# Sunsett5/Noise-space-HMC

Measured on AMD Instinct MI355X. Metric: HMC leapfrog chain-steps/sec (256x256x3 FFHQ inpaint_random, U-Net score in the loop), higher is better.
Workload: dtype f32; 1 GPU; BASELINE configs[1]: FFHQ 256x256 inpaint_random sigma_0=0.05 tau=1.0 eps=0.05 timesteps=3, 64 chains per GPU, FFHQ U-Net architecture random-init fp32; chains_per_gpu=64, global_chains=64, score_chunk=64, parallelism=chains sharded over 1 rank(s), no data-path collective

## Files before the change

### noise-space-hmc_amd/csrc/wino_conv.hip

```cpp
#include "nhmc_common.h"

namespace {

typedef float f32x16 __attribute__((ext_vector_type(16)));
typedef float wc_v2f __attribute__((ext_vector_type(2)));

constexpr int WC_KBLK = 64;
constexpr int WC_ROWS = 4, WC_COLS = 64;
constexpr int WC_CHUNK = 8;
constexpr int WC_OPER = 16 * WC_CHUNK * 64;
constexpr int WC_LDS_BYTES = 4 * WC_OPER * 4;

#ifdef NHMC_WINO_STAMPS
__device__ unsigned long long* nhmc_wino_stamps;
__device__ int nhmc_wino_stamp_chunk;
#define WC_FENCE() __builtin_amdgcn_sched_barrier(0)
#define WC_T64(i) do { WC_FENCE(); t64[i] = __builtin_amdgcn_s_memtime(); WC_FENCE(); } while (0)
#define WC_R64(i) do { WC_FENCE(); t64[i] = __builtin_amdgcn_s_memrealtime(); WC_FENCE(); } while (0)
#define WC_T32(i) do { WC_FENCE(); const unsigned now_ = (unsigned)__builtin_amdgcn_s_memtime(); \
                       t32[i] = ch == stamp_ch ? now_ : t32[i]; WC_FENCE(); } while (0)
#else
#define WC_T64(i)
#define WC_R64(i)
#define WC_T32(i)
#endif

struct WinoArgs {
  const float* x; const float* U; const float* bias; const float* add; float* y;
  int C, K, H, W, row_blocks, col_blocks;
};

template <int TC, bool TAIL>
__global__ __launch_bounds__(256, 1) void k_conv3x3_wino(const WinoArgs a) {
  static_assert(TC == 32 || TC == 16 || TC == 8, "64 tiles as 32 / TC row pairs x TC columns");
  constexpr int BLK_ROWS = 128 / TC, BLK_COLS = 2 * TC;
  extern __shared__ __attribute__((aligned(16))) float lds[];
  const int tid = threadIdx.x, lane = tid & 63, wave = tid >> 6, lr = lane & 31, lh = lane >> 5;
  const int kh = wave & 1, th = wave >> 1;
  const int C = a.C, K = a.K, H = a.H, W = a.W, HW = H * W;
#ifdef NHMC_WINO_STAMPS
  unsigned long long t64[7] = {};
  unsigned t32[13] = {};
  const int stamp_ch = nhmc_wino_stamp_chunk < C / WC_CHUNK ? nhmc_wino_stamp_chunk : C / WC_CHUNK - 1;
#endif
  WC_T64(0);

  const int total = gridDim.x;
  int logical = blockIdx.x;
  if ((total & 7) == 0) logical = (logical & 7) * (total >> 3) + (logical >> 3);
  const int kblocks = TAIL ? (K + WC_KBLK - 1) / WC_KBLK : K / WC_KBLK;
  const int kb = logical % kblocks, sp = logical / kblocks;
  const bool tail_block = TAIL && kb == kblocks - 1;
  const bool idle = tail_block && __builtin_amdgcn_readfirstlane(kh) == 1;
  const bool u_row_ok = !(tail_block && tid >= 128);
  const int cb = sp % a.col_blocks, rb = (sp / a.col_blocks) % a.row_blocks, n = sp / (a.col_blocks * a.row_blocks);
  const int h0 = rb * BLK_ROWS, w0 = cb * BLK_COLS;

  const int lc = tid >> 5, ltx = tid & 31;
  unsigned voff[6][4];
  unsigned okmask = 0;
#pragma unroll
  for (int r = 0; r < 6; ++r) {
    const int row = h0 + 4 * (ltx / TC) - 1 + r;
    const bool rok = (unsigned)row < (unsigned)H;
#pragma unroll
    for (int s = 0; s < 4; ++s) {
      const int col = w0 + 2 * (ltx % TC) - 1 + s;
      const bool ok = rok && (unsigned)col < (unsigned)W;
      voff[r][s] = ok ? 4u * (unsigned)(lc * HW + row * W + col) : 0u;
      okmask |= ok ? 1u << (r * 4 + s) : 0u;
    }
  }
  const float* xn = a.x + (int64_t)n * C * HW;
  const char* un = reinterpret_cast<const char*>(a.U + (int64_t)kb * WC_KBLK * 16);
  const unsigned uoff = 16u * tid;
  const int uw = (tid & ~3) * 4 + (((tid & 3) ^ ((tid >> 4) & 3)) << 2);
  const int vw = (lc * 64 + ltx) * 16, vswz = (ltx >> 2) & 3;

  float xr[6][4];
  nhmc_v4f ur[8];
  auto load_one = [&](int ch, int i) {
    if (i < 24) {
      const char* xs = reinterpret_cast<const char*>(xn + (int64_t)ch * WC_CHUNK * HW);
      unsigned off = voff[i >> 2][i & 3];
      asm volatile("" : "+v"(off));
      xr[i >> 2][i & 3] = *reinterpret_cast<const float*>(xs + off);
    } else {
      const char* us = un + (int64_t)ch * WC_CHUNK * K * 64 + (int64_t)(i - 24) * K * 64;
      unsigned off = uoff;
      asm volatile("" : "+v"(off));
      if (!TAIL || u_row_ok) ur[i - 24] = *reinterpret_cast<const nhmc_v4f*>(us + off);
      else ur[i - 24] = nhmc_v4f{0.0f, 0.0f, 0.0f, 0.0f};
    }
  };
  auto issue_loads = [&](int ch, int first, int last) {
#pragma unroll
    for (int i = first; i < last; ++i) load_one(ch, i);
  };
  auto pin_patch = [&]() {
#pragma unroll
    for (int r = 0; r < 6; ++r)
#pragma unroll
      for (int s = 0; s < 4; ++s) asm volatile("" : "+v"(xr[r][s]));
  };
  auto d = [&](int r, int s) { return (okmask >> (r * 4 + s)) & 1u ? xr[r][s] : 0.0f; };
  auto stage_part = [&](int st, int b) {
    float* Us = lds + st * 2 * WC_OPER;
    float* Vs = Us + WC_OPER;
    float e[6];
#pragma unroll
    for (int r = 0; r < 6; ++r)
      e[r] = b == 0 ? d(r, 0) - d(r, 2) : b == 1 ? d(r, 1) + d(r, 2) : b == 2 ? d(r, 2) - d(r, 1) : d(r, 1) - d(r, 3);
#pragma unroll
    for (int ty = 0; ty < 2; ++ty) {
      const int r0 = 2 * ty;
      nhmc_v4f v;
      v.x = e[r0] - e[r0 + 2]; v.y = e[r0 + 1] + e[r0 + 2]; v.z = e[r0 + 2] - e[r0 + 1]; v.w = e[r0 + 1] - e[r0 + 3];
      *reinterpret_cast<nhmc_v4f*>(Vs + vw + ty * 32 * 16 + ((b ^ vswz) << 2)) = v;
    }
#pragma unroll
    for (int i = 2 * b; i < 2 * b + 2; ++i) *reinterpret_cast<nhmc_v4f*>(Us + uw + 1024 * i) = ur[i];
  };

  const int chunks = C / WC_CHUNK;
  f32x16 acc[16];
#pragma unroll
  for (int f = 0; f < 16; ++f)
#pragma unroll
    for (int r = 0; r < 16; ++r) acc[f][r] = 0.0f;

  const int swz = (lr >> 2) & 3;
  const int arow = (lh * 64 + kh * 32 + lr) * 16, brow = WC_OPER + (lh * 64 + th * 32 + lr) * 16;
  float av[2][8], bv[2][8];
  auto fetch = [&](int st, int u, float (&fa)[8], float (&fb)[8]) {
    const float* S = lds + st * 2 * WC_OPER + (u >> 1) * 2 * 64 * 16;
#pragma unroll
    for (int g = 0; g < 2; ++g) {
      const int go = ((2 * (u & 1) + g) ^ swz) << 2;
      const nhmc_v4f va = *reinterpret_cast<const nhmc_v4f*>(S + arow + go);
      const nhmc_v4f vb = *reinterpret_cast<const nhmc_v4f*>(S + brow + go);
      fa[4 * g + 0] = va.x; fa[4 * g + 1] = va.y; fa[4 * g + 2] = va.z; fa[4 * g + 3] = va.w;
      fb[4 * g + 0] = vb.x; fb[4 * g + 1] = vb.y; fb[4 * g + 2] = vb.z; fb[4 * g + 3] = vb.w;
    }
  };
  auto unit = [&](int u) {
#pragma unroll
    for (int j = 0; j < 8; ++j) {
      const int f = 8 * (u & 1) + j;
      if (!TAIL || !idle) acc[f] = __builtin_amdgcn_mfma_f32_32x32x2f32(av[u & 1][j], bv[u & 1][j], acc[f], 0, 0, 0);
    }
  };
  auto unit_loading = [&](int u, int cl) {
#pragma unroll
    for (int j = 0; j < 8; ++j) {
      const int f = 8 * (u & 1) + j;
      if (!TAIL || !idle) acc[f] = __builtin_amdgcn_mfma_f32_32x32x2f32(av[u & 1][j], bv[u & 1][j], acc[f], 0, 0, 0);
      if (u == 7) issue_loads(cl, (3 * j) / 2, (3 * j + 3) / 2);
      if (u == 0 && j < 6) issue_loads(cl, 12 + 2 * j, 14 + 2 * j);
      if (u == 0 && j >= 6) issue_loads(cl, 18 + j, 19 + j);
      if (u == 1 && (j & 1) == 0) issue_loads(cl, 26 + j / 2, 27 + j / 2);
      if (u == 2 && (j == 0 || j == 2)) issue_loads(cl, 30 + j / 2, 31 + j / 2);
      __builtin_amdgcn_sched_barrier(0);
    }
  };

  issue_loads(0, 0, 32);
#pragma unroll
  for (int b = 0; b < 4; ++b) stage_part(0, b);
  __syncthreads();
  WC_T64(1);
  int cl = 1 < chunks ? 1 : 0;
  issue_loads(cl, 0, 12);
  fetch(0, 0, av[0], bv[0]);
  int ch = 0, st = 0;
  WC_T64(2);
  WC_R64(5);
  do {
#pragma unroll
    for (int u = 0; u < 7; ++u) {
      WC_T32(u);
      fetch(st, u + 1, av[(u + 1) & 1], bv[(u + 1) & 1]);
      __builtin_amdgcn_sched_barrier(0);
      if (u < 3) unit_loading(u, cl);
      else unit(u);
      if (u == 3) {
        WC_T32(7);
        pin_patch();
        WC_T32(8);
      }
      if (u >= 3) stage_part(st ^ 1, u - 3);
    }
    WC_T32(9);
    __syncthreads();
    WC_T32(10);
    st ^= 1;
    cl = ch + 2 < chunks ? ch + 2 : chunks - 1;
    WC_T32(11);
    fetch(st, 0, av[0], bv[0]);
    __builtin_amdgcn_sched_barrier(0);
    unit_loading(7, cl);
    WC_T32(12);
  } while (++ch < chunks);
  WC_T64(3);
  WC_R64(6);

  if (TAIL && idle) return;
  const int oh = h0 + 4 * (lr / TC) + 2 * th, ow = w0 + 2 * (lr % TC);
  const bool has_bias = a.bias != nullptr, has_add = a.add != nullptr;
  const int k0 = kb * WC_KBLK + kh * 32 + 4 * lh;
  const bool odd = lr & 1;
  const int64_t at0 = (((int64_t)n * K + k0) * H + oh) * W + ow + (odd ? W - 2 : 0);
  float bc[16];
  nhmc_v4f ad[16];
#pragma unroll
  for (int r = 0; r < 16; ++r) {
    bc[r] = 0.0f;
    ad[r] = nhmc_v4f{0.0f, 0.0f, 0.0f, 0.0f};
  }
  if (has_bias) {
#pragma unroll
    for (int r = 0; r < 16; ++r) bc[r] = a.bias[k0 + (r & 3) + 8 * (r >> 2)];
  }
  if (has_add) {
#pragma unroll
    for (int r = 0; r < 16; ++r)
      ad[r] = *reinterpret_cast<const nhmc_v4f*>(a.add + at0 + (int64_t)((r & 3) + 8 * (r >> 2)) * HW);
  }
  auto neighbour = [](float v) {
    return __int_as_float(__builtin_amdgcn_update_dpp(0, __float_as_int(v), 0xB1, 0xF, 0xF, false));
  };
  __builtin_amdgcn_sched_barrier(0);
#pragma unroll
  for (int r = 0; r < 16; ++r) {
    float t[2][4];
#pragma unroll
    for (int b = 0; b < 4; ++b) {
      t[0][b] = (acc[4 * b + 0][r] + acc[4 * b + 1][r]) + acc[4 * b + 2][r];
      t[1][b] = (acc[4 * b + 1][r] - acc[4 * b + 2][r]) - acc[4 * b + 3][r];
    }
    wc_v2f o[2];
#pragma unroll
    for (int i = 0; i < 2; ++i) {
      o[i].x = (t[i][0] + t[i][1]) + t[i][2];
      o[i].y = (t[i][1] - t[i][2]) - t[i][3];
      o[i].x = has_bias ? o[i].x + bc[r] : o[i].x;
      o[i].y = has_bias ? o[i].y + bc[r] : o[i].y;
    }
    const wc_v2f keep = odd ? o[1] : o[0], send = odd ? o[0] : o[1];
    const wc_v2f got = {neighbour(send.x), neighbour(send.y)};
    nhmc_v4f v;
    v.x = odd ? got.x : keep.x; v.y = odd ? got.y : keep.y; v.z = odd ? keep.x : got.x; v.w = odd ? keep.y : got.y;
    if (has_add) v += ad[r];
    __builtin_nontemporal_store(v, reinterpret_cast<nhmc_v4f*>(a.y + at0 + (int64_t)((r & 3) + 8 * (r >> 2)) * HW));
  }
  WC_T64(4);
#ifdef NHMC_WINO_STAMPS
  if (nhmc_wino_stamps && lane == 0) {
    unsigned long long* out = nhmc_wino_stamps + ((size_t)blockIdx.x * 4 + wave) * 24;
#pragma unroll
    for (int i = 0; i < 7; ++i) out[i] = t64[i];
#pragma unroll
    for (int i = 0; i < 13; ++i) out[7 + i] = t32[i];
  }
#endif
}

__global__ __launch_bounds__(NHMC_BLOCK) void k_wino_weights(const float* __restrict__ w, float* __restrict__ U, int C, int K,
                                                             int backward) {
  const int CI = backward ? K : C, KO = backward ? C : K;
  const int idx = blockIdx.x * NHMC_BLOCK + threadIdx.x;
  if (idx >= CI * KO) return;
  const int ci = idx / KO, ko = idx % KO;
  const float* g = w + (int64_t)(backward ? ci * C + ko : ko * C + ci) * 9;
  float t[4][3];
#pragma unroll
  for (int s = 0; s < 3; ++s) {
    const float g0 = g[backward ? 8 - s : s], g1 = g[backward ? 5 - s : 3 + s], g2 = g[backward ? 2 - s : 6 + s];
    t[0][s] = g0; t[1][s] = 0.5f * ((g0 + g1) + g2); t[2][s] = 0.5f * ((g0 - g1) + g2); t[3][s] = g2;
  }
  nhmc_v4f u[4];
#pragma unroll
  for (int r = 0; r < 4; ++r) {
    u[0][r] = t[r][0];
    u[1][r] = 0.5f * ((t[r][0] + t[r][1]) + t[r][2]);
    u[2][r] = 0.5f * ((t[r][0] - t[r][1]) + t[r][2]);
    u[3][r] = t[r][2];
  }
#pragma unroll
  for (int b = 0; b < 4; ++b) reinterpret_cast<nhmc_v4f*>(U + (int64_t)idx * 16)[b] = u[b];
}

template <int TC, int KM = WC_KBLK>
int wc_covers_tc(int64_t n, int64_t c, int64_t k, int64_t h, int64_t w) {
  constexpr int ROWS = 128 / TC, COLS = 2 * TC;
  if (n <= 0 || c < WC_CHUNK || c % WC_CHUNK || k < KM || k % KM || h < ROWS || h % ROWS || w < COLS || w % COLS)
    return 0;
  if (TC != 32 && w != COLS) return 0;
  if (c > 65536 || k > 65536 || h * w > (1 << 24)) return 0;
  return n * (h / ROWS) * (w / COLS) * ((k + WC_KBLK - 1) / WC_KBLK) < (int64_t)1 << 31;
}

int wc_covers(int64_t n, int64_t c, int64_t k, int64_t h, int64_t w) { return wc_covers_tc<32>(n, c, k, h, w); }

int wc_narrow_covers(int64_t n, int64_t c, int64_t k, int64_t h, int64_t w) {
  return w == 32 ? wc_covers_tc<16>(n, c, k, h, w) : w == 16 ? wc_covers_tc<8>(n, c, k, h, w) : 0;
}

int wc_k32_covers(int64_t n, int64_t c, int64_t k, int64_t h, int64_t w) {
  return w == 32 ? wc_covers_tc<16, 32>(n, c, k, h, w) : w == 16 ? wc_covers_tc<8, 32>(n, c, k, h, w)
                                                                 : wc_covers_tc<32, 32>(n, c, k, h, w);
}

static_assert(WC_ROWS == 128 / 32 && WC_COLS == 2 * 32, "the wide geometry");

struct WcRow { int backward, c, k, res; };

template <int N>
int wc_listed(const WcRow (&table)[N], int backward, int c, int k, int h) {
  for (const WcRow& r : table)
    if (r.backward == (backward != 0) && r.c == c && r.k == k && r.res == h) return 1;
  return 0;
}

template <int TC, bool TAIL = false>
int wc_launch(const float* x, const float* u, const float* bias, const float* add, float* y, int n, int c, int k, int h, int w,
              nhmc_stream_t stream) {
  static bool attr_set[64] = {};
  int dev = 0;
  (void)hipGetDevice(&dev);
  if (dev < 0 || dev >= 64 || !attr_set[dev]) {
    if (hipFuncSetAttribute(reinterpret_cast<const void*>(&k_conv3x3_wino<TC, TAIL>), hipFuncAttributeMaxDynamicSharedMemorySize,
                            WC_LDS_BYTES) != hipSuccess)
      return NHMC_ERR_LAUNCH;
    if (dev >= 0 && dev < 64) attr_set[dev] = true;
  }
  const WinoArgs a{x, u, bias, add, y, c, k, h, w, h / (128 / TC), w / (2 * TC)};
  const int64_t blocks = (int64_t)n * a.row_blocks * a.col_blocks * ((k + WC_KBLK - 1) / WC_KBLK);
  NHMC_LAUNCH((k_conv3x3_wino<TC, TAIL>), dim3((unsigned)blocks), dim3(256), WC_LDS_BYTES, nhmc_s(stream), a);
  return nhmc_launch_status();
}

}

extern "C" int nhmc_conv3x3_wino_covers(int n, int c, int k, int h, int w) { return wc_covers(n, c, k, h, w); }
extern "C" int nhmc_conv3x3_wino_narrow_covers(int n, int c, int k, int h, int w) { return wc_narrow_covers(n, c, k, h, w); }

extern "C" int nhmc_conv3x3_wino_prefers(int backward, int n, int c, int k, int h, int w) {
  if (!wc_covers(n, c, k, h, w) || h != w) return 0;
  static const WcRow network[] = {
      {0, 128, 128, 256},
      {1, 128, 128, 256},
      {0, 256, 128, 256},
      {1, 128, 256, 256},
      {0, 128, 128, 128},
      {1, 128, 128, 128},
      {0, 256, 128, 128},
      {1, 128, 256, 128},
      {0, 256, 256, 128},
      {1, 256, 256, 128},
      {0, 384, 128, 128},
      {1, 128, 384, 128},
      {0, 128, 128, 64},
      {1, 128, 128, 64},
      {0, 128, 256, 64},
      {1, 256, 128, 64},
      {0, 256, 256, 64},
      {1, 256, 256, 64},
      {0, 384, 256, 64},
      {1, 256, 384, 64},
      {0, 512, 256, 64},
      {1, 256, 512, 64},
  };
  static const WcRow elsewhere[] = {
      {0, 384, 128, 256},
      {1, 128, 384, 256},
      {0, 128, 256, 128},
      {1, 256, 128, 128},
      {0, 384, 256, 128},
      {1, 256, 384, 128},
      {0, 512, 256, 128},
      {1, 256, 512, 128},
      {0, 256, 512, 64},
      {1, 512, 256, 64},
      {0, 512, 512, 64},
      {1, 512, 512, 64},
      {0, 768, 256, 64},
      {1, 256, 768, 64},
      {0, 1024, 512, 64},
      {1, 512, 1024, 64},
  };
  static const WcRow latent[] = {
      {0, 448, 448, 64},
      {0, 256, 256, 256},
      {1, 256, 256, 256},
      {0, 512, 512, 128},
      {1, 512, 512, 128},
  };
  return wc_listed(network, backward, c, k, h) || wc_listed(elsewhere, backward, c, k, h) || wc_listed(latent, backward, c, k, h);
}

extern "C" int nhmc_conv3x3_wino_narrow_prefers(int backward, int n, int c, int k, int h, int w) {
  if (!wc_narrow_covers(n, c, k, h, w) || h != w) return 0;
  static const WcRow network[] = {
      {0, 256, 256, 32},
      {1, 256, 256, 32},
      {0, 512, 256, 32},
      {1, 256, 512, 32},
      {0, 512, 512, 32},
      {1, 512, 512, 32},
      {0, 768, 256, 32},
      {1, 256, 768, 32},
      {0, 256, 256, 16},
      {1, 256, 256, 16},
      {0, 256, 512, 16},
      {1, 512, 256, 16},
      {0, 512, 512, 16},
      {1, 512, 512, 16},
      {0, 768, 512, 16},
      {1, 512, 768, 16},
      {0, 1024, 512, 16},
      {1, 512, 1024, 16},
  };
  static const WcRow latent[] = {
      {0, 224, 448, 32},
      {0, 448, 448, 32},
      {0, 672, 448, 32},
      {0, 896, 448, 32},
      {0, 1120, 448, 32},
      {0, 896, 896, 16},
  };
  return wc_listed(network, backward, c, k, h) || wc_listed(latent, backward, c, k, h);
}

extern "C" int nhmc_conv3x3_wino_k32_covers(int n, int c, int k, int h, int w) { return wc_k32_covers(n, c, k, h, w); }

extern "C" int nhmc_conv3x3_wino_k32_prefers(int backward, int n, int c, int k, int h, int w) {
  if (!wc_k32_covers(n, c, k, h, w) || h != w || k % WC_KBLK == 0) return 0;
  static const WcRow latent[] = {
      {0, 224, 224, 64},
      {0, 448, 224, 64},
      {0, 672, 224, 64},
      {0, 672, 672, 32},
      {0, 448, 672, 16},
      {0, 672, 672, 16},
      {0, 1120, 672, 16},
      {0, 1344, 672, 16},
      {0, 1568, 672, 16},
  };
  return wc_listed(latent, backward, c, k, h);
}

extern "C" int nhmc_wino_weights(const float* weight, float* u, int backward, int channels_in, int channels_out,
                                 nhmc_stream_t stream) {
  if (!weight || !u || (backward != 0 && backward != 1) || channels_in <= 0 || channels_out <= 0) return NHMC_ERR_ARG;
  if (channels_in > 65536 || channels_out > 65536) return NHMC_ERR_SHAPE;
  if (!nhmc_aligned16(u)) return NHMC_ERR_ALIGN;
  const int pairs = channels_in * channels_out;
  NHMC_LAUNCH(k_wino_weights, dim3((unsigned)((pairs + NHMC_BLOCK - 1) / NHMC_BLOCK)), dim3(NHMC_BLOCK), 0, nhmc_s(stream), weight,
              u, channels_in, channels_out, backward);
  return nhmc_launch_status();
}

extern "C" int nhmc_conv3x3_wino(const float* x, const float* u, const float* bias, const float* add, float* y, int n, int c,
                                 int k, int h, int w, int stride, int padding, nhmc_stream_t stream) {
  if (!x || !u || !y || y == x || (add && add == x)) return NHMC_ERR_ARG;
  if (stride != 1 || padding != 1 || !wc_covers(n, c, k, h, w)) return NHMC_ERR_SHAPE;
  if (!nhmc_aligned16(x) || !nhmc_aligned16(u) || !nhmc_aligned16(y) || !nhmc_aligned16(add)) return NHMC_ERR_ALIGN;
  return wc_launch<32>(x, u, bias, add, y, n, c, k, h, w, stream);
}

extern "C" int nhmc_conv3x3_wino_narrow(const float* x, const float* u, const float* bias, const float* add, float* y, int n,
                                        int c, int k, int h, int w, int stride, int padding, nhmc_stream_t stream) {
  if (!x || !u || !y || y == x || (add && add == x)) return NHMC_ERR_ARG;
  if (stride != 1 || padding != 1 || !wc_narrow_covers(n, c, k, h, w)) return NHMC_ERR_SHAPE;
  if (!nhmc_aligned16(x) || !nhmc_aligned16(u) || !nhmc_aligned16(y) || !nhmc_aligned16(add)) return NHMC_ERR_ALIGN;
  return w == 32 ? wc_launch<16>(x, u, bias, add, y, n, c, k, h, w, stream)
                 : wc_launch<8>(x, u, bias, add, y, n, c, k, h, w, stream);
}

extern "C" int nhmc_conv3x3_wino_k32(const float* x, const float* u, const float* bias, const float* add, float* y, int n, int c,
                                     int k, int h, int w, int stride, int padding, nhmc_stream_t stream) {
  if (!x || !u || !y || y == x || (add && add == x)) return NHMC_ERR_ARG;
  if (stride != 1 || padding != 1 || !wc_k32_covers(n, c, k, h, w)) return NHMC_ERR_SHAPE;
  if (!nhmc_aligned16(x) || !nhmc_aligned16(u) || !nhmc_aligned16(y) || !nhmc_aligned16(add)) return NHMC_ERR_ALIGN;
  if (k % WC_KBLK == 0)
    return w == 32   ? wc_launch<16>(x, u, bias, add, y, n, c, k, h, w, stream)
           : w == 16 ? wc_launch<8>(x, u, bias, add, y, n, c, k, h, w, stream)
                     : wc_launch<32>(x, u, bias, add, y, n, c, k, h, w, stream);
  return w == 32   ? wc_launch<16, true>(x, u, bias, add, y, n, c, k, h, w, stream)
         : w == 16 ? wc_launch<8, true>(x, u, bias, add, y, n, c, k, h, w, stream)
                   : wc_launch<32, true>(x, u, bias, add, y, n, c, k, h, w, stream);
}
```

Measured before the change: 63.16 chain-steps/s.

## Load Winograd input patches as float2 with DPP neighbour exchange and interleave staging

Each thread now loads its two central patch columns as one float2 per row and gets its left and right neighbour columns from adjacent lanes through DPP row shifts. Only edge lanes issue an extra scalar load, and only for TC=32. This cuts the per-chunk global patch loads from 24 scalar loads to 6 or 12, and frees VGPRs. The LDS transform and staging work is also split into pieces interleaved between individual MFMAs, and the LDS swizzle gets a new XOR pattern to reduce bank conflicts. The risk is that DPP shifts at lane-row boundaries give wrong neighbours when TC is below 16, and the tighter hand scheduling could add stalls.

```diff
diff --git a/noise-space-hmc_amd/csrc/wino_conv.hip b/noise-space-hmc_amd/csrc/wino_conv.hip
--- a/noise-space-hmc_amd/csrc/wino_conv.hip
+++ b/noise-space-hmc_amd/csrc/wino_conv.hip
@@ -10,6 +10,8 @@
 constexpr int WC_CHUNK = 8;
 constexpr int WC_OPER = 16 * WC_CHUNK * 64;
 constexpr int WC_LDS_BYTES = 4 * WC_OPER * 4;
+
+__device__ __forceinline__ constexpr int wc_swz(int R) { return ((R >> 1) & 3) ^ (((R >> 3) & 1) ? 3 : 0); }
 
 #ifdef NHMC_WINO_STAMPS
 __device__ unsigned long long* nhmc_wino_stamps;
@@ -40,7 +42,7 @@
   const int C = a.C, K = a.K, H = a.H, W = a.W, HW = H * W;
 #ifdef NHMC_WINO_STAMPS
   unsigned long long t64[7] = {};
-  unsigned t32[13] = {};
+  unsigned t32[17] = {};
   const int stamp_ch = nhmc_wino_stamp_chunk < C / WC_CHUNK ? nhmc_wino_stamp_chunk : C / WC_CHUNK - 1;
 #endif
   WC_T64(0);
@@ -56,41 +58,49 @@
   const int cb = sp % a.col_blocks, rb = (sp / a.col_blocks) % a.row_blocks, n = sp / (a.col_blocks * a.row_blocks);
   const int h0 = rb * BLK_ROWS, w0 = cb * BLK_COLS;
 
-  const int lc = tid >> 5, ltx = tid & 31;
-  unsigned voff[6][4];
+  constexpr bool EDGE = TC == 32;
+  constexpr int NP = EDGE ? 12 : 6;
+  const int lc = tid >> 5, ltx = tid & 31, lt = ltx % TC;
+  unsigned voff[6], eoff[6];
   unsigned okmask = 0;
+  const int ecol = lt == 0 ? w0 - 1 : w0 + 2 * TC;
+  const bool eok = EDGE && (lt == 0 || lt == TC - 1) && (unsigned)ecol < (unsigned)W;
 #pragma unroll
   for (int r = 0; r < 6; ++r) {
     const int row = h0 + 4 * (ltx / TC) - 1 + r;
     const bool rok = (unsigned)row < (unsigned)H;
+    voff[r] = rok ? 4u * (unsigned)(lc * HW + row * W + w0 + 2 * lt) : 0u;
+    eoff[r] = rok ? 4u * (unsigned)(lc * HW + row * W + (eok ? ecol : w0 + 2 * lt)) : 0u;
 #pragma unroll
     for (int s = 0; s < 4; ++s) {
-      const int col = w0 + 2 * (ltx % TC) - 1 + s;
+      const int col = w0 + 2 * lt - 1 + s;
       const bool ok = rok && (unsigned)col < (unsigned)W;
-      voff[r][s] = ok ? 4u * (unsigned)(lc * HW + row * W + col) : 0u;
       okmask |= ok ? 1u << (r * 4 + s) : 0u;
     }
   }
   const float* xn = a.x + (int64_t)n * C * HW;
   const char* un = reinterpret_cast<const char*>(a.U + (int64_t)kb * WC_KBLK * 16);
   const unsigned uoff = 16u * tid;
-  const int uw = (tid & ~3) * 4 + (((tid & 3) ^ ((tid >> 4) & 3)) << 2);
-  const int vw = (lc * 64 + ltx) * 16, vswz = (ltx >> 2) & 3;
-
-  float xr[6][4];
+  const int uw = (tid & ~3) * 4 + (((tid & 3) ^ wc_swz(tid >> 2)) << 2);
+  const int vw = (lc * 64 + ltx) * 16, vswz = wc_swz(ltx);
+
+  wc_v2f xm[6];
+  float xl[6], xq[6], xe[6];
   nhmc_v4f ur[8];
   auto load_one = [&](int ch, int i) {
-    if (i < 24) {
+    if (i < NP) {
       const char* xs = reinterpret_cast<const char*>(xn + (int64_t)ch * WC_CHUNK * HW);
-      unsigned off = voff[i >> 2][i & 3];
+      const int r = EDGE ? i >> 1 : i;
+      unsigned off = EDGE && (i & 1) ? eoff[r] : voff[r];
       asm volatile("" : "+v"(off));
-      xr[i >> 2][i & 3] = *reinterpret_cast<const float*>(xs + off);
+      if (EDGE && (i & 1)) xe[r] = *reinterpret_cast<const float*>(xs + off);
+      else xm[r] = *reinterpret_cast<const wc_v2f*>(xs + off);
     } else {
-      const char* us = un + (int64_t)ch * WC_CHUNK * K * 64 + (int64_t)(i - 24) * K * 64;
+      const char* us = un + (int64_t)ch * WC_CHUNK * K * 64 + (int64_t)(i - NP) * K * 64;
       unsigned off = uoff;
       asm volatile("" : "+v"(off));
-      if (!TAIL || u_row_ok) ur[i - 24] = *reinterpret_cast<const nhmc_v4f*>(us + off);
-      else ur[i - 24] = nhmc_v4f{0.0f, 0.0f, 0.0f, 0.0f};
+      if (!TAIL || u_row_ok) ur[i - NP] = *reinterpret_cast<const nhmc_v4f*>(us + off);
+      else ur[i - NP] = nhmc_v4f{0.0f, 0.0f, 0.0f, 0.0f};
     }
   };
   auto issue_loads = [&](int ch, int first, int last) {
@@ -99,27 +109,52 @@
   };
   auto pin_patch = [&]() {
 #pragma unroll
-    for (int r = 0; r < 6; ++r)
-#pragma unroll
-      for (int s = 0; s < 4; ++s) asm volatile("" : "+v"(xr[r][s]));
-  };
-  auto d = [&](int r, int s) { return (okmask >> (r * 4 + s)) & 1u ? xr[r][s] : 0.0f; };
-  auto stage_part = [&](int st, int b) {
-    float* Us = lds + st * 2 * WC_OPER;
-    float* Vs = Us + WC_OPER;
-    float e[6];
-#pragma unroll
-    for (int r = 0; r < 6; ++r)
+    for (int r = 0; r < 6; ++r) {
+      asm volatile("" : "+v"(xm[r]));
+      if (EDGE) asm volatile("" : "+v"(xe[r]));
+    }
+  };
+  auto exchange_patch = [&]() {
+#pragma unroll
+    for (int r = 0; r < 6; ++r) {
+      xl[r] = __int_as_float(__builtin_amdgcn_update_dpp(0, __float_as_int(xm[r].y), 0x138, 0xF, 0xF, false));
+      xq[r] = __int_as_float(__builtin_amdgcn_update_dpp(0, __float_as_int(xm[r].x), 0x130, 0xF, 0xF, false));
+      if (EDGE) {
+        xl[r] = lt == 0 ? xe[r] : xl[r];
+        xq[r] = lt == TC - 1 ? xe[r] : xq[r];
+      }
+    }
+  };
+  auto d = [&](int r, int s) {
+    const float v = s == 0 ? xl[r] : s == 1 ? xm[r].x : s == 2 ? xm[r].y : xq[r];
+    return (okmask >> (r * 4 + s)) & 1u ? v : 0.0f;
+  };
+  float e[6];
+  auto stage_rows = [&](int b, int first, int last) {
+#pragma unroll
+    for (int r = first; r < last; ++r)
       e[r] = b == 0 ? d(r, 0) - d(r, 2) : b == 1 ? d(r, 1) + d(r, 2) : b == 2 ? d(r, 2) - d(r, 1) : d(r, 1) - d(r, 3);
+  };
+  nhmc_v4f vt[2];
+  auto stage_cols = [&]() {
 #pragma unroll
     for (int ty = 0; ty < 2; ++ty) {
       const int r0 = 2 * ty;
-      nhmc_v4f v;
-      v.x = e[r0] - e[r0 + 2]; v.y = e[r0 + 1] + e[r0 + 2]; v.z = e[r0 + 2] - e[r0 + 1]; v.w = e[r0 + 1] - e[r0 + 3];
-      *reinterpret_cast<nhmc_v4f*>(Vs + vw + ty * 32 * 16 + ((b ^ vswz) << 2)) = v;
-    }
-#pragma unroll
-    for (int i = 2 * b; i < 2 * b + 2; ++i) *reinterpret_cast<nhmc_v4f*>(Us + uw + 1024 * i) = ur[i];
+      vt[ty].x = e[r0] - e[r0 + 2]; vt[ty].y = e[r0 + 1] + e[r0 + 2]; vt[ty].z = e[r0 + 2] - e[r0 + 1]; vt[ty].w = e[r0 + 1] - e[r0 + 3];
+    }
+  };
+  auto stage_v = [&](int st, int b, int ty) {
+    float* Vs = lds + st * 2 * WC_OPER + WC_OPER;
+    *reinterpret_cast<nhmc_v4f*>(Vs + vw + ty * 32 * 16 + ((b ^ vswz) << 2)) = vt[ty];
+  };
+  auto stage_u = [&](int st, int i) { *reinterpret_cast<nhmc_v4f*>(lds + st * 2 * WC_OPER + uw + 1024 * i) = ur[i]; };
+  auto stage_part = [&](int st, int b) {
+    stage_rows(b, 0, 6);
+    stage_cols();
+    stage_v(st, b, 0);
+    stage_v(st, b, 1);
+    stage_u(st, 2 * b);
+    stage_u(st, 2 * b + 1);
   };
 
   const int chunks = C / WC_CHUNK;
@@ -129,48 +164,66 @@
 #pragma unroll
     for (int r = 0; r < 16; ++r) acc[f][r] = 0.0f;
 
-  const int swz = (lr >> 2) & 3;
+  const int swz = wc_swz(lr);
   const int arow = (lh * 64 + kh * 32 + lr) * 16, brow = WC_OPER + (lh * 64 + th * 32 + lr) * 16;
   float av[2][8], bv[2][8];
+  auto fetch_half = [&](int st, int u, int g, float (&fa)[8], float (&fb)[8]) {
+    const float* S = lds + st * 2 * WC_OPER + (u >> 1) * 2 * 64 * 16;
+    const int go = ((2 * (u & 1) + g) ^ swz) << 2;
+    const nhmc_v4f va = *reinterpret_cast<const nhmc_v4f*>(S + arow + go);
+    const nhmc_v4f vb = *reinterpret_cast<const nhmc_v4f*>(S + brow + go);
+    fa[4 * g + 0] = va.x; fa[4 * g + 1] = va.y; fa[4 * g + 2] = va.z; fa[4 * g + 3] = va.w;
+    fb[4 * g + 0] = vb.x; fb[4 * g + 1] = vb.y; fb[4 * g + 2] = vb.z; fb[4 * g + 3] = vb.w;
+  };
   auto fetch = [&](int st, int u, float (&fa)[8], float (&fb)[8]) {
-    const float* S = lds + st * 2 * WC_OPER + (u >> 1) * 2 * 64 * 16;
-#pragma unroll
-    for (int g = 0; g < 2; ++g) {
-      const int go = ((2 * (u & 1) + g) ^ swz) << 2;
-      const nhmc_v4f va = *reinterpret_cast<const nhmc_v4f*>(S + arow + go);
-      const nhmc_v4f vb = *reinterpret_cast<const nhmc_v4f*>(S + brow + go);
-      fa[4 * g + 0] = va.x; fa[4 * g + 1] = va.y; fa[4 * g + 2] = va.z; fa[4 * g + 3] = va.w;
-      fb[4 * g + 0] = vb.x; fb[4 * g + 1] = vb.y; fb[4 * g + 2] = vb.z; fb[4 * g + 3] = vb.w;
-    }
-  };
-  auto unit = [&](int u) {
+    fetch_half(st, u, 0, fa, fb);
+    fetch_half(st, u, 1, fa, fb);
+  };
+  auto unit_loading = [&](int u, int cl) {
 #pragma unroll
     for (int j = 0; j < 8; ++j) {
       const int f = 8 * (u & 1) + j;
       if (!TAIL || !idle) acc[f] = __builtin_amdgcn_mfma_f32_32x32x2f32(av[u & 1][j], bv[u & 1][j], acc[f], 0, 0, 0);
-    }
-  };
-  auto unit_loading = [&](int u, int cl) {
+      if (u == 7) issue_loads(cl, (NP / 2 * j) / 8, (NP / 2 * (j + 1)) / 8);
+      if (u == 0 && j < 6) issue_loads(cl, NP / 2 + (NP / 2 * j) / 6, NP / 2 + (NP / 2 * (j + 1)) / 6);
+      if (u == 0 && j >= 6) issue_loads(cl, NP - 6 + j, NP - 5 + j);
+      if (u == 1 && (j & 1) == 0) issue_loads(cl, NP + 2 + j / 2, NP + 3 + j / 2);
+      if (u == 2 && (j == 0 || j == 2)) issue_loads(cl, NP + 6 + j / 2, NP + 7 + j / 2);
+      __builtin_amdgcn_sched_barrier(0);
+    }
+  };
+
+  auto unit_staging = [&](int u, int st, int ch) {
+    const int b = u - 3;
 #pragma unroll
     for (int j = 0; j < 8; ++j) {
       const int f = 8 * (u & 1) + j;
+      if (u == 4 && (j & 1)) WC_T32(13 + j / 2);
       if (!TAIL || !idle) acc[f] = __builtin_amdgcn_mfma_f32_32x32x2f32(av[u & 1][j], bv[u & 1][j], acc[f], 0, 0, 0);
-      if (u == 7) issue_loads(cl, (3 * j) / 2, (3 * j + 3) / 2);
-      if (u == 0 && j < 6) issue_loads(cl, 12 + 2 * j, 14 + 2 * j);
-      if (u == 0 && j >= 6) issue_loads(cl, 18 + j, 19 + j);
-      if (u == 1 && (j & 1) == 0) issue_loads(cl, 26 + j / 2, 27 + j / 2);
-      if (u == 2 && (j == 0 || j == 2)) issue_loads(cl, 30 + j / 2, 31 + j / 2);
+      if (j == 0 && u == 3) {
+        WC_T32(7);
+        pin_patch();
+        exchange_patch();
+        WC_T32(8);
+      }
+      if (j < 2) fetch_half(st, u + 1, j, av[(u + 1) & 1], bv[(u + 1) & 1]);
+      if (j == 1) stage_rows(b, 0, 3);
+      if (j == 2) stage_rows(b, 3, 6);
+      if (j == 3) stage_cols();
+      if (j == 3 || j == 4) stage_v(st ^ 1, b, j - 3);
+      if (j == 5 || j == 6) stage_u(st ^ 1, 2 * b + j - 5);
       __builtin_amdgcn_sched_barrier(0);
     }
   };
 
-  issue_loads(0, 0, 32);
+  issue_loads(0, 0, NP + 8);
+  exchange_patch();
 #pragma unroll
   for (int b = 0; b < 4; ++b) stage_part(0, b);
   __syncthreads();
   WC_T64(1);
   int cl = 1 < chunks ? 1 : 0;
-  issue_loads(cl, 0, 12);
+  issue_loads(cl, 0, NP / 2);
   fetch(0, 0, av[0], bv[0]);
   int ch = 0, st = 0;
   WC_T64(2);
@@ -179,16 +232,13 @@
 #pragma unroll
     for (int u = 0; u < 7; ++u) {
       WC_T32(u);
-      fetch(st, u + 1, av[(u + 1) & 1], bv[(u + 1) & 1]);
-      __builtin_amdgcn_sched_barrier(0);
-      if (u < 3) unit_loading(u, cl);
-      else unit(u);
-      if (u == 3) {
-        WC_T32(7);
-        pin_patch();
-        WC_T32(8);
+      if (u < 3) {
+        fetch(st, u + 1, av[(u + 1) & 1], bv[(u + 1) & 1]);
+        __builtin_amdgcn_sched_barrier(0);
+        unit_loading(u, cl);
+      } else {
+        unit_staging(u, st, ch);
       }
-      if (u >= 3) stage_part(st ^ 1, u - 3);
     }
     WC_T32(9);
     __syncthreads();
@@ -260,7 +310,7 @@
 #pragma unroll
     for (int i = 0; i < 7; ++i) out[i] = t64[i];
 #pragma unroll
-    for (int i = 0; i < 13; ++i) out[7 + i] = t32[i];
+    for (int i = 0; i < 17; ++i) out[7 + i] = t32[i];
   }
 #endif
 }
```

Result: faster. 69.57 chain-steps/s (median of 6 runs) (+10.1%).
